# tusen-ai/SST

Hardware: AMD Instinct MI355X
Metric: LiDAR frames/sec (SST backbone fwd+bwd) at Waymo 0.32m voxels (higher is better)
Workload: dtype f32 (storage, accumulation, attention, LayerNorm, reductions: fp32; the dense products of the encoder layers from the EXACT three-way bf16 split of both fp32 operands, six bf16 MFMA products with fp32 accumulation - error vs float64 <= 2 x the fp32 matrix pipe's: tests/test_gpu_dense_f32x6.py)

## Files before the change

### sst_amd/csrc/wgrad_x6.hip

```cpp
#include <math.h>
#include <stdlib.h>
#include "common.h"

namespace {

typedef float f32x4 __attribute__((ext_vector_type(4)));
typedef float f32x2 __attribute__((ext_vector_type(2)));
typedef unsigned u32x4 __attribute__((ext_vector_type(4)));
typedef unsigned u32x2 __attribute__((ext_vector_type(2)));
typedef __bf16 bf16x8 __attribute__((ext_vector_type(8)));
typedef __bf16 bf16x2 __attribute__((ext_vector_type(2)));

__device__ __forceinline__ unsigned pack2(float lo, float hi) {
  const f32x2 v = {lo, hi};
  return __builtin_bit_cast(unsigned, __builtin_convertvector(v, bf16x2));
}
__device__ __forceinline__ float lo_f(unsigned p) { return __uint_as_float(p << 16); }
__device__ __forceinline__ float hi_f(unsigned p) { return __uint_as_float(p & 0xffff0000u); }
__device__ __forceinline__ f32x4 mma32(u32x4 a, u32x4 b, f32x4 c) {
  return __builtin_amdgcn_mfma_f32_16x16x32_bf16(__builtin_bit_cast(bf16x8, a), __builtin_bit_cast(bf16x8, b), c, 0, 0, 0);
}
__device__ __forceinline__ void split2(float a, float b, unsigned& p0, unsigned& p1, unsigned& p2) {
  p0 = pack2(a, b);
  const float ra = a - lo_f(p0), rb = b - hi_f(p0);
  p1 = pack2(ra, rb);
  p2 = pack2(ra - lo_f(p1), rb - hi_f(p1));
}

constexpr int kMaxProblems = 8;
constexpr int kTile = 128;
constexpr int kStep = 32;
constexpr int kTileLds = 1040;
constexpr int kImage = 8 * kTileLds;
constexpr int kStage = 2 * 3 * kImage;
constexpr int kLdsBytes = 2 * kStage;

struct x6_problem {
  const float* dy;
  const float* x;
  int64_t m, ld_dy, ld_x;
  int out, in;
  int tile0;
  int db_off;
  float* dw;
  float* db;
  const float* x_add_rows;
  const int32_t* x_add_index;
};
struct x6_group {
  x6_problem p[kMaxProblems];
  int n, tiles, slices;
  int64_t tokens_per_slice;
};

__global__ __launch_bounds__(512, 2) void wgrad_x6_k(const x6_group G, float* __restrict__ part, float* __restrict__ dbp) {
  extern __shared__ __attribute__((aligned(16))) unsigned char lds[];
  const int tid = threadIdx.x, lane = tid & 63, wave = tid >> 6;
  const int l15 = lane & 15, g = lane >> 4;
  const int tile = blockIdx.x / G.slices, slice = blockIdx.x - tile * G.slices;
  int pi = 0;
#pragma unroll
  for (int q = 1; q < kMaxProblems; ++q)
    if (q < G.n && tile >= G.p[q].tile0) pi = q;
  const x6_problem P = G.p[pi];
  const int tiles_k = P.in / kTile;
  const int tl = tile - P.tile0, tn = tl / tiles_k, tk = tl - tn * tiles_k;
  const int n0 = tn * kTile, k0 = tk * kTile;
  const int64_t t_begin = (int64_t)slice * G.tokens_per_slice;
  int64_t t_end = t_begin + G.tokens_per_slice;
  t_end = t_end < P.m ? t_end : P.m;

  const int op = tid >> 8, tq = (tid >> 5) & 7, cg = tid & 31;
  const float* src = op == 0 ? P.dy + n0 + 4 * cg : P.x + k0 + 4 * cg;
  const int64_t ld = op == 0 ? P.ld_dy : P.ld_x;
  const int st_off = (cg >> 2) * kTileLds + (tq & 1) * 512 + (tq >> 1) * 128 + (cg & 3) * 32;
  constexpr int kPf = 2;
  f32x4 rows[kPf][4];
  const int64_t t_last = t_end > 0 ? t_end - 1 : 0;
  const bool xadd = op == 1 && P.x_add_rows != nullptr;
  const float* addsrc = xadd ? P.x_add_rows + k0 + 4 * cg : nullptr;
  f32x4 prow[kPf][4];
  int32_t pidx[4] = {0, 0, 0, 0};
  auto load_idx = [&](int64_t t0) {
#pragma unroll
    for (int r = 0; r < 4; ++r) {
      int64_t t = t0 + 4 * tq + r;
      t = t < t_last ? t : t_last;
      pidx[r] = P.x_add_index[t];
    }
  };
  auto load_rows = [&](int64_t t0, f32x4 (&dst)[4], f32x4 (&pdst)[4]) {
#pragma unroll
    for (int r = 0; r < 4; ++r) {
      int64_t t = t0 + 4 * tq + r;
      t = t < t_last ? t : t_last;
      dst[r] = *(const f32x4*)(src + t * ld);
    }
    if (xadd) {
#pragma unroll
      for (int r = 0; r < 4; ++r) pdst[r] = *(const f32x4*)(addsrc + (int64_t)pidx[r] * P.in);
      load_idx(t0 + kStep);
    }
  };
  float bsum[4] = {0.f, 0.f, 0.f, 0.f};
  u32x4 img[3][2];
  auto split_col = [&](int e, int64_t t0, const f32x4 (&rws)[4], const f32x4 (&prw)[4]) {
    float v[4];
#pragma unroll
    for (int r = 0; r < 4; ++r) v[r] = (t0 + 4 * tq + r < t_end) ? (xadd ? rws[r][e] + prw[r][e] : rws[r][e]) : 0.f;
    if (op == 0) bsum[e] += (v[0] + v[1]) + (v[2] + v[3]);
    unsigned a0, a1, a2, b0, b1, b2;
    split2(v[0], v[1], a0, a1, a2);
    split2(v[2], v[3], b0, b1, b2);
    img[0][e >> 1][2 * (e & 1)] = a0;
    img[0][e >> 1][2 * (e & 1) + 1] = b0;
    img[1][e >> 1][2 * (e & 1)] = a1;
    img[1][e >> 1][2 * (e & 1) + 1] = b1;
    img[2][e >> 1][2 * (e & 1)] = a2;
    img[2][e >> 1][2 * (e & 1) + 1] = b2;
  };
  auto store_img = [&](int buf) {
    unsigned char* base = lds + buf * kStage + op * 3 * kImage + st_off;
#pragma unroll
    for (int im = 0; im < 3; ++im) {
      *(u32x4*)(base + im * kImage) = img[im][0];
      *(u32x4*)(base + im * kImage + 16) = img[im][1];
    }
  };
  const int wn = wave & 3, wk = wave >> 2;
  const int frag_off = g * 128 + l15 * 8;
  f32x4 acc[4][2], acl[4][2];
#pragma unroll
  for (int a = 0; a < 4; ++a)
#pragma unroll
    for (int b = 0; b < 2; ++b) acc[a][b] = acl[a][b] = (f32x4){0.f, 0.f, 0.f, 0.f};
  auto frag = [&](const unsigned char* image, int tile16) -> u32x4 {
    const unsigned char* p = image + tile16 * kTileLds + frag_off;
    const u32x2 lo = *(const u32x2*)p, hi = *(const u32x2*)(p + 512);
    return (u32x4){lo[0], lo[1], hi[0], hi[1]};
  };

  if (xadd) load_idx(t_begin);
#pragma unroll
  for (int u = 0; u < kPf; ++u) load_rows(t_begin + (int64_t)u * kStep, rows[u], prow[u]);
#pragma unroll
  for (int e = 0; e < 4; ++e) split_col(e, t_begin, rows[0], prow[0]);
  store_img(0);
  load_rows(t_begin + (int64_t)kPf * kStep, rows[0], prow[0]);
  __syncthreads();
  const int64_t n_steps = (t_end - t_begin + kStep - 1) / kStep;
  for (int64_t s0 = 0; s0 < n_steps; s0 += kPf) {
#pragma unroll
    for (int u = 0; u < kPf; ++u) {
      const int64_t s = s0 + u;
      if (s >= n_steps) break;
      const int64_t t1 = t_begin + (s + 1) * kStep;
      const unsigned char* dyi = lds + (u & 1) * kStage;
      const unsigned char* xi = dyi + 3 * kImage;
      u32x4 b0[2], b1[2], b2[2];
#pragma unroll
      for (int b = 0; b < 2; ++b) {
        b0[b] = frag(dyi, 2 * wn + b);
        b1[b] = frag(dyi + kImage, 2 * wn + b);
        b2[b] = frag(dyi + 2 * kImage, 2 * wn + b);
      }
#pragma unroll
      for (int a = 0; a < 4; ++a) {
        const u32x4 a0 = frag(xi, 4 * wk + a), a1 = frag(xi + kImage, 4 * wk + a), a2 = frag(xi + 2 * kImage, 4 * wk + a);
#pragma unroll
        for (int b = 0; b < 2; ++b) acl[a][b] = mma32(a2, b0[b], acl[a][b]);
#pragma unroll
        for (int b = 0; b < 2; ++b) acl[a][b] = mma32(a0, b2[b], acl[a][b]);
#pragma unroll
        for (int b = 0; b < 2; ++b) acl[a][b] = mma32(a1, b1[b], acl[a][b]);
#pragma unroll
        for (int b = 0; b < 2; ++b) acl[a][b] = mma32(a1, b0[b], acl[a][b]);
#pragma unroll
        for (int b = 0; b < 2; ++b) acl[a][b] = mma32(a0, b1[b], acl[a][b]);
#pragma unroll
        for (int b = 0; b < 2; ++b) acc[a][b] = mma32(a0, b0[b], acc[a][b]);
        split_col(a, t1, rows[(u + 1) % kPf], prow[(u + 1) % kPf]);
      }
      store_img((u + 1) & 1);
      load_rows(t1 + (int64_t)kPf * kStep, rows[(u + 1) % kPf], prow[(u + 1) % kPf]);
      __syncthreads();
    }
  }
#pragma unroll
  for (int a = 0; a < 4; ++a)
#pragma unroll
    for (int b = 0; b < 2; ++b) acc[a][b] += acl[a][b];
  float* dst = part + ((int64_t)tile * G.slices + slice) * (kTile * kTile);
#pragma unroll
  for (int a = 0; a < 4; ++a)
#pragma unroll
    for (int b = 0; b < 2; ++b)
      *(f32x4*)(dst + (32 * wn + 16 * b + l15) * kTile + 64 * wk + 16 * a + 4 * g) = acc[a][b];
  if (P.db_off >= 0 && tk == 0) {
    float* red = (float*)lds;
    if (op == 0) *(f32x4*)(red + tq * 128 + 4 * cg) = (f32x4){bsum[0], bsum[1], bsum[2], bsum[3]};
    __syncthreads();
    if (tid < 128) {
      float s = 0.f;
#pragma unroll
      for (int q = 0; q < 8; ++q) s += red[q * 128 + tid];
      dbp[((int64_t)P.db_off + n0 + tid) * G.slices + slice] = s;
    }
  }
}

struct x6_riders {
  sst_colsum_rider r[2];
  int n, blocks0;
};

constexpr int kRedQuads = 32, kRedGroups = 8;

__global__ __launch_bounds__(256) void wgrad_x6_reduce_k(const x6_group G, const float* __restrict__ part,
                                                         const float* __restrict__ dbp, int rider_blocks,
                                                         const x6_riders R) {
  __shared__ double red[kRedGroups][kRedQuads][4];
  if ((int)blockIdx.x < rider_blocks) {
    const int second = (int)blockIdx.x >= R.blocks0 ? 1 : 0;
    const sst_colsum_rider& J = R.r[second];
    const int rblk = (int)blockIdx.x - (second ? R.blocks0 : 0);
    float* fr = (float*)&red[0][0][0];
    const int cx = threadIdx.x & 31, gq = threadIdx.x >> 5;
    const int i = rblk * 32 + cx;
    float acc[4] = {0.f, 0.f, 0.f, 0.f};
    if (i < J.width) {
      const float* src = J.partials + i;
      for (int base = 0; base < J.nb; base += 512) {
        float v[16][4];
#pragma unroll
        for (int it = 0; it < 16; ++it)
#pragma unroll
          for (int j = 0; j < 4; ++j) {
            const int b = base + 32 * it + gq + 8 * j;
            v[it][j] = src[(int64_t)(b < J.nb ? b : J.nb - 1) * J.width];
          }
#pragma unroll
        for (int it = 0; it < 16; ++it)
#pragma unroll
          for (int j = 0; j < 4; ++j)
            if (base + 32 * it + gq + 8 * j < J.nb) acc[j] += v[it][j];
      }
    }
#pragma unroll
    for (int j = 0; j < 4; ++j) fr[(gq + 8 * j) * 33 + cx] = acc[j];
    __syncthreads();
    if (gq == 0 && i < J.width) {
      float t = 0.f;
#pragma unroll
      for (int k = 0; k < 32; ++k) t += fr[k * 33 + cx];
      if (i < J.split)
        J.out0[i] = t;
      else
        J.out1[i - J.split] = t;
    }
    return;
  }
  const int blk = (int)blockIdx.x - rider_blocks;
  const int ql = threadIdx.x & (kRedQuads - 1), sg = threadIdx.x / kRedQuads;
  const int64_t quad = (int64_t)blk * kRedQuads + ql;
  const int64_t tile = quad / (kTile * kTile / 4);
  const int e4 = (int)(quad - tile * (kTile * kTile / 4));
  double d0 = 0.0, d1 = 0.0, d2 = 0.0, d3 = 0.0;
  if (tile < G.tiles) {
    const float* src = part + tile * G.slices * (int64_t)(kTile * kTile) + 4 * e4;
#pragma unroll 8
    for (int q = sg; q < G.slices; q += kRedGroups) {
      const f32x4 v = *(const f32x4*)(src + (int64_t)q * (kTile * kTile));
      d0 += v[0], d1 += v[1], d2 += v[2], d3 += v[3];
    }
  }
  red[sg][ql][0] = d0, red[sg][ql][1] = d1, red[sg][ql][2] = d2, red[sg][ql][3] = d3;
  __syncthreads();
  if (sg == 0 && tile < G.tiles) {
    f32x4 s;
#pragma unroll
    for (int r = 0; r < 4; ++r) {
      double t = 0.0;
#pragma unroll
      for (int k = 0; k < kRedGroups; ++k) t += red[k][ql][r];
      s[r] = (float)t;
    }
    int pi = 0;
#pragma unroll
    for (int q = 1; q < kMaxProblems; ++q)
      if (q < G.n && tile >= G.p[q].tile0) pi = q;
    const int tiles_k = G.p[pi].in / kTile;
    const int tl = (int)tile - G.p[pi].tile0, tn = tl / tiles_k, tk = tl - tn * tiles_k;
    const int n = tn * kTile + e4 / 32, k = tk * kTile + (e4 % 32) * 4;
    *(f32x4*)(G.p[pi].dw + (int64_t)n * G.p[pi].in + k) = s;
  }
  const int64_t col = (int64_t)blk * 256 + threadIdx.x;
  int base = 0;
  for (int q = 0; q < G.n; ++q) {
    if (G.p[q].db_off < 0) continue;
    if (col >= base && col < base + G.p[q].out) {
      const float* src = dbp + ((int64_t)G.p[q].db_off + (col - base)) * G.slices;
      double s = 0.0;
      for (int i = 0; i < G.slices; ++i) s += src[i];
      G.p[q].db[col - base] = (float)s;
    }
    base += G.p[q].out;
  }
}

bool aligned16(const void* p) { return ((uintptr_t)p & 15) == 0; }

struct x6_plan {
  x6_group g;
  int64_t part_bytes, db_bytes;
};

bool make_plan(const sst_wgrad_problem_f32* pr, int n, x6_plan* plan) {
  if (!pr || n < 1 || n > kMaxProblems) return false;
  x6_group& G = plan->g;
  G.n = n;
  int tiles = 0, db_cols = 0;
  int64_t m = pr[0].m;
  for (int i = 0; i < n; ++i) {
    const sst_wgrad_problem_f32& p = pr[i];
    if (p.m != m || p.m < 1 || p.out < kTile || p.in < kTile || (p.out % kTile) || (p.in % kTile) || (p.ld_dy & 3) ||
        (p.ld_x & 3) || !p.dy || !p.x || !p.dw || !aligned16(p.dy) || !aligned16(p.x) || !aligned16(p.dw))
      return false;
    G.p[i].dy = p.dy;
    G.p[i].x = p.x;
    G.p[i].m = p.m;
    G.p[i].ld_dy = p.ld_dy;
    G.p[i].ld_x = p.ld_x;
    G.p[i].out = p.out;
    G.p[i].in = p.in;
    G.p[i].tile0 = tiles;
    G.p[i].db_off = p.db ? db_cols : -1;
    G.p[i].dw = p.dw;
    G.p[i].db = p.db;
    if ((p.x_add_rows != nullptr) != (p.x_add_index != nullptr) || (p.x_add_rows && !aligned16(p.x_add_rows))) return false;
    G.p[i].x_add_rows = p.x_add_rows;
    G.p[i].x_add_index = p.x_add_index;
    tiles += (p.out / kTile) * (p.in / kTile);
    if (p.db) db_cols += p.out;
  }
  G.tiles = tiles;
  int slices = (256 / tiles) & ~7;
  if (slices < 8) slices = 8;
  const int64_t max_slices = sst_div_up(m, (int64_t)kStep);
  while (slices > 8 && slices > max_slices) slices -= 8;
  G.slices = slices;
  G.tokens_per_slice = sst_align_up(sst_div_up(m, (int64_t)slices), (int64_t)kStep);
  plan->part_bytes = sst_align_up((int64_t)tiles * slices * kTile * kTile * 4, 256);
  plan->db_bytes = sst_align_up((int64_t)(db_cols > 0 ? db_cols : 1) * slices * 4, 256);
  return true;
}

}

extern "C" {

int64_t sst_weight_grad_group_f32x6_workspace_bytes(const sst_wgrad_problem_f32* problems, int n) {
  x6_plan plan;
  if (!make_plan(problems, n, &plan)) return SST_ERR_UNSUPPORTED;
  return plan.part_bytes + plan.db_bytes;
}

}

int sst_internal_weight_grad_group_f32x6(const sst_wgrad_problem_f32* problems, int n, void* d_workspace,
                                         const sst_colsum_rider* riders, int n_riders, void* stream) {
  x6_plan plan;
  if (!make_plan(problems, n, &plan)) return SST_ERR_UNSUPPORTED;
  if (!d_workspace || !aligned16(d_workspace)) return SST_ERR_ARG;
  hipStream_t st = (hipStream_t)stream;
  float* part = (float*)d_workspace;
  float* dbp = (float*)((char*)d_workspace + plan.part_bytes);
  static unsigned long long configured = 0;
  if (sst_first_use_on_device(&configured)) {
    SST_HIP(hipFuncSetAttribute((const void*)wgrad_x6_k, hipFuncAttributeMaxDynamicSharedMemorySize, kLdsBytes));
    sst_mark_device(&configured);
  }
  const int64_t quads = (int64_t)plan.g.tiles * (kTile * kTile / 4);
  const int tile_blocks = (int)sst_div_up(quads, (int64_t)kRedQuads);
  if (n_riders < 0 || n_riders > 2 || (n_riders > 0 && !riders)) return SST_ERR_ARG;
  x6_riders R;
  R.n = n_riders, R.blocks0 = 0;
  int extra = 0;
  for (int i = 0; i < n_riders; ++i) {
    const sst_colsum_rider& q = riders[i];
    if (!q.partials || q.nb < 1 || q.width < 1 || !q.out0 || !q.out1) return SST_ERR_ARG;
    R.r[i] = q;
    if (i == 0) R.blocks0 = (q.width + 31) / 32;
    extra += (q.width + 31) / 32;
  }
  hipLaunchKernelGGL(wgrad_x6_k, dim3((unsigned)(plan.g.tiles * plan.g.slices)), dim3(512), kLdsBytes, st, plan.g, part, dbp);
  hipLaunchKernelGGL(wgrad_x6_reduce_k, dim3((unsigned)(tile_blocks + extra)), dim3(256), 0, st, plan.g, part, dbp, extra, R);
  SST_LAUNCH_CHECK();
  return SST_OK;
}

extern "C" {

int sst_weight_grad_group_f32x6(const sst_wgrad_problem_f32* problems, int n, void* d_workspace, void* stream) {
  return sst_internal_weight_grad_group_f32x6(problems, n, d_workspace, nullptr, 0, stream);
}

}
```

Measured before the change: 97.71.

## Add warp-specialized wgrad x6 path and buffer loads, swizzled LDS, unmasked steps

Adds an optional producer/consumer variant of the x6 weight-gradient kernel in which 8 waves only run MFMAs while 4 extra waves load, split and stage both operands. It is selected by an environment variable and off by default. The default path also changes: full steps use buffer loads with scalar offsets and skip bounds masking, the LDS image layout is XOR-swizzled with permlane32 swaps so fragments load as one 16-byte read, and the bias sum runs only where it is needed. These aim to cut address arithmetic, masking and LDS bank conflicts, at the cost of code complexity and a separate ragged tail loop.

```diff
diff --git a/sst_amd/csrc/wgrad_x6.hip b/sst_amd/csrc/wgrad_x6.hip
--- a/sst_amd/csrc/wgrad_x6.hip
+++ b/sst_amd/csrc/wgrad_x6.hip
@@ -1,5 +1,6 @@
 #include <math.h>
 #include <stdlib.h>
+#include <type_traits>
 #include "common.h"
 
 namespace {
@@ -25,6 +26,15 @@
   const float ra = a - lo_f(p0), rb = b - hi_f(p0);
   p1 = pack2(ra, rb);
   p2 = pack2(ra - lo_f(p1), rb - hi_f(p1));
+}
+
+__device__ __forceinline__ __amdgpu_buffer_rsrc_t row_block(const void* p) {
+  const uint64_t v = (uint64_t)p;
+  const unsigned lo = __builtin_amdgcn_readfirstlane((unsigned)v), hi = __builtin_amdgcn_readfirstlane((unsigned)(v >> 32));
+  return __builtin_amdgcn_make_buffer_rsrc((void*)(((uint64_t)hi << 32) | lo), 0, 0x7fffffff, 0x00020000);
+}
+__device__ __forceinline__ f32x4 load16(__amdgpu_buffer_rsrc_t rs, unsigned voff, unsigned soff) {
+  return __builtin_bit_cast(f32x4, __builtin_amdgcn_raw_buffer_load_b128(rs, (int)voff, (int)soff, 0));
 }
 
 constexpr int kMaxProblems = 8;
@@ -34,6 +44,7 @@
 constexpr int kImage = 8 * kTileLds;
 constexpr int kStage = 2 * 3 * kImage;
 constexpr int kLdsBytes = 2 * kStage;
+constexpr bool kRolesDefault = false;
 
 struct x6_problem {
   const float* dy;
@@ -53,62 +64,101 @@
   int64_t tokens_per_slice;
 };
 
-__global__ __launch_bounds__(512, 2) void wgrad_x6_k(const x6_group G, float* __restrict__ part, float* __restrict__ dbp) {
+template <bool kRoles>
+__global__ __launch_bounds__(kRoles ? 768 : 512, kRoles ? 3 : 2) void wgrad_x6_k(const x6_group G, float* __restrict__ part,
+                                                                                 float* __restrict__ dbp) {
   extern __shared__ __attribute__((aligned(16))) unsigned char lds[];
-  const int tid = threadIdx.x, lane = tid & 63, wave = tid >> 6;
+  const int tid = threadIdx.x, lane = tid & 63;
+  const int wave = __builtin_amdgcn_readfirstlane(tid >> 6);
   const int l15 = lane & 15, g = lane >> 4;
-  const int tile = blockIdx.x / G.slices, slice = blockIdx.x - tile * G.slices;
+  const int tile = __builtin_amdgcn_readfirstlane(blockIdx.x / G.slices), slice = blockIdx.x - tile * G.slices;
   int pi = 0;
 #pragma unroll
   for (int q = 1; q < kMaxProblems; ++q)
     if (q < G.n && tile >= G.p[q].tile0) pi = q;
   const x6_problem P = G.p[pi];
   const int tiles_k = P.in / kTile;
-  const int tl = tile - P.tile0, tn = tl / tiles_k, tk = tl - tn * tiles_k;
+  const int tl = tile - P.tile0, tn = __builtin_amdgcn_readfirstlane(tl / tiles_k), tk = tl - tn * tiles_k;
   const int n0 = tn * kTile, k0 = tk * kTile;
   const int64_t t_begin = (int64_t)slice * G.tokens_per_slice;
   int64_t t_end = t_begin + G.tokens_per_slice;
   t_end = t_end < P.m ? t_end : P.m;
 
-  const int op = tid >> 8, tq = (tid >> 5) & 7, cg = tid & 31;
-  const float* src = op == 0 ? P.dy + n0 + 4 * cg : P.x + k0 + 4 * cg;
-  const int64_t ld = op == 0 ? P.ld_dy : P.ld_x;
-  const int st_off = (cg >> 2) * kTileLds + (tq & 1) * 512 + (tq >> 1) * 128 + (cg & 3) * 32;
+  constexpr int kOps = kRoles ? 2 : 1;
+  const int op0 = kRoles ? 0 : wave >> 2;
+  const int tq = (tid >> 5) & 7, cg = tid & 31;
+  const float* opbase[kOps];
+  int64_t ld[kOps];
+  unsigned voff[kOps][4];
+  __amdgpu_buffer_rsrc_t rs[kOps];
+#pragma unroll
+  for (int o = 0; o < kOps; ++o) {
+    opbase[o] = op0 + o == 0 ? P.dy + n0 : P.x + k0;
+    ld[o] = op0 + o == 0 ? P.ld_dy : P.ld_x;
+    rs[o] = row_block(opbase[o] + t_begin * ld[o]);
+#pragma unroll
+    for (int r = 0; r < 4; ++r) voff[o][r] = (unsigned)((4 * tq + r) * ld[o] * 4 + 16 * cg);
+  }
+  const int st_col = 4 * (cg & 3) + 2 * (tq & 1);
+  const int st_off = (cg >> 2) * kTileLds + (tq >> 1) * 256 + (st_col ^ ((st_col & 8) >> 2)) * 16;
   constexpr int kPf = 2;
-  f32x4 rows[kPf][4];
+  constexpr int kPp = kRoles ? 1 : kPf;
+  f32x4 rows[kPf][kOps][4];
   const int64_t t_last = t_end > 0 ? t_end - 1 : 0;
-  const bool xadd = op == 1 && P.x_add_rows != nullptr;
+  constexpr int oX = kRoles ? 1 : 0;
+  const bool xadd = op0 + oX == 1 && P.x_add_rows != nullptr;
   const float* addsrc = xadd ? P.x_add_rows + k0 + 4 * cg : nullptr;
-  f32x4 prow[kPf][4];
+  f32x4 prow[kPp][4];
   int32_t pidx[4] = {0, 0, 0, 0};
-  auto load_idx = [&](int64_t t0) {
+  const __amdgpu_buffer_rsrc_t idx_rs = row_block(xadd ? P.x_add_index + t_begin : nullptr);
+  auto load_idx = [&](auto full, int64_t j) {
+    const int64_t t0 = t_begin + j * kStep;
 #pragma unroll
     for (int r = 0; r < 4; ++r) {
-      int64_t t = t0 + 4 * tq + r;
-      t = t < t_last ? t : t_last;
-      pidx[r] = P.x_add_index[t];
-    }
-  };
-  auto load_rows = [&](int64_t t0, f32x4 (&dst)[4], f32x4 (&pdst)[4]) {
-#pragma unroll
-    for (int r = 0; r < 4; ++r) {
-      int64_t t = t0 + 4 * tq + r;
-      t = t < t_last ? t : t_last;
-      dst[r] = *(const f32x4*)(src + t * ld);
-    }
+      if constexpr (decltype(full)::value) {
+        pidx[r] = (int32_t)__builtin_amdgcn_raw_buffer_load_b32(idx_rs, 4 * (4 * tq + r), (int)(j * kStep * 4), 0);
+      } else {
+        int64_t t = t0 + 4 * tq + r;
+        t = t < t_last ? t : t_last;
+        pidx[r] = P.x_add_index[t];
+      }
+    }
+  };
+  auto load_rows = [&](auto full, int64_t j, f32x4 (&dst)[kOps][4]) {
+    const int64_t t0 = t_begin + j * kStep;
+#pragma unroll
+    for (int o = 0; o < kOps; ++o) {
+      if constexpr (decltype(full)::value) {
+#pragma unroll
+        for (int r = 0; r < 4; ++r) dst[o][r] = load16(rs[o], voff[o][r], (unsigned)(j * kStep * ld[o] * 4));
+      } else {
+#pragma unroll
+        for (int r = 0; r < 4; ++r) {
+          int64_t t = t0 + 4 * tq + r;
+          t = t < t_last ? t : t_last;
+          dst[o][r] = *(const f32x4*)(opbase[o] + t * ld[o] + 4 * cg);
+        }
+      }
+    }
+  };
+  auto load_pos = [&](auto full, int64_t j, f32x4 (&pdst)[4]) {
     if (xadd) {
 #pragma unroll
       for (int r = 0; r < 4; ++r) pdst[r] = *(const f32x4*)(addsrc + (int64_t)pidx[r] * P.in);
-      load_idx(t0 + kStep);
-    }
-  };
+      load_idx(full, j + 1);
+    }
+  };
+  const bool want_b = P.db_off >= 0 && tk == 0;
   float bsum[4] = {0.f, 0.f, 0.f, 0.f};
   u32x4 img[3][2];
-  auto split_col = [&](int e, int64_t t0, const f32x4 (&rws)[4], const f32x4 (&prw)[4]) {
+  auto split_col = [&](auto full, int e, int o, int64_t j, const f32x4 (&rws)[4], const f32x4 (&prw)[4]) {
     float v[4];
 #pragma unroll
-    for (int r = 0; r < 4; ++r) v[r] = (t0 + 4 * tq + r < t_end) ? (xadd ? rws[r][e] + prw[r][e] : rws[r][e]) : 0.f;
-    if (op == 0) bsum[e] += (v[0] + v[1]) + (v[2] + v[3]);
+    for (int r = 0; r < 4; ++r) {
+      v[r] = (o == oX && xadd) ? rws[r][e] + prw[r][e] : rws[r][e];
+      if constexpr (!decltype(full)::value) v[r] = (t_begin + j * kStep + 4 * tq + r < t_end) ? v[r] : 0.f;
+    }
+    if (op0 + o == 0 && want_b) bsum[e] += (v[0] + v[1]) + (v[2] + v[3]);
     unsigned a0, a1, a2, b0, b1, b2;
     split2(v[0], v[1], a0, a1, a2);
     split2(v[2], v[3], b0, b1, b2);
@@ -119,86 +169,146 @@
     img[2][e >> 1][2 * (e & 1)] = a2;
     img[2][e >> 1][2 * (e & 1) + 1] = b2;
   };
-  auto store_img = [&](int buf) {
-    unsigned char* base = lds + buf * kStage + op * 3 * kImage + st_off;
+  auto store_img = [&](int buf, int o) {
+    unsigned char* base = lds + buf * kStage + (op0 + o) * 3 * kImage + st_off;
 #pragma unroll
     for (int im = 0; im < 3; ++im) {
-      *(u32x4*)(base + im * kImage) = img[im][0];
-      *(u32x4*)(base + im * kImage + 16) = img[im][1];
-    }
-  };
-  const int wn = wave & 3, wk = wave >> 2;
-  const int frag_off = g * 128 + l15 * 8;
+      u32x2 w[4];
+#pragma unroll
+      for (int i = 0; i < 4; ++i) w[i] = __builtin_amdgcn_permlane32_swap(img[im][0][i], img[im][1][i], false, false);
+      *(u32x4*)(base + im * kImage) = (u32x4){w[0][0], w[1][0], w[0][1], w[1][1]};
+      *(u32x4*)(base + im * kImage + 16) = (u32x4){w[2][0], w[3][0], w[2][1], w[3][1]};
+    }
+  };
+  const int wn = wave & 3, wk = (wave >> 2) & 1;
+  const int frag_off = g * 256 + (l15 ^ ((l15 & 8) >> 2)) * 16;
   f32x4 acc[4][2], acl[4][2];
-#pragma unroll
-  for (int a = 0; a < 4; ++a)
-#pragma unroll
-    for (int b = 0; b < 2; ++b) acc[a][b] = acl[a][b] = (f32x4){0.f, 0.f, 0.f, 0.f};
+  auto zero_acc = [&]() {
+#pragma unroll
+    for (int a = 0; a < 4; ++a)
+#pragma unroll
+      for (int b = 0; b < 2; ++b) acc[a][b] = acl[a][b] = (f32x4){0.f, 0.f, 0.f, 0.f};
+  };
   auto frag = [&](const unsigned char* image, int tile16) -> u32x4 {
     const unsigned char* p = image + tile16 * kTileLds + frag_off;
-    const u32x2 lo = *(const u32x2*)p, hi = *(const u32x2*)(p + 512);
-    return (u32x4){lo[0], lo[1], hi[0], hi[1]};
-  };
-
-  if (xadd) load_idx(t_begin);
-#pragma unroll
-  for (int u = 0; u < kPf; ++u) load_rows(t_begin + (int64_t)u * kStep, rows[u], prow[u]);
-#pragma unroll
-  for (int e = 0; e < 4; ++e) split_col(e, t_begin, rows[0], prow[0]);
-  store_img(0);
-  load_rows(t_begin + (int64_t)kPf * kStep, rows[0], prow[0]);
-  __syncthreads();
+    return *(const u32x4*)p;
+  };
+  auto multiply = [&](int buf, auto&& between) {
+    const unsigned char* dyi = lds + buf * kStage;
+    const unsigned char* xi = dyi + 3 * kImage;
+    u32x4 b0[2], b1[2], b2[2];
+#pragma unroll
+    for (int b = 0; b < 2; ++b) {
+      b0[b] = frag(dyi, 2 * wn + b);
+      b1[b] = frag(dyi + kImage, 2 * wn + b);
+      b2[b] = frag(dyi + 2 * kImage, 2 * wn + b);
+    }
+#pragma unroll
+    for (int a = 0; a < 4; ++a) {
+      const u32x4 a0 = frag(xi, 4 * wk + a), a1 = frag(xi + kImage, 4 * wk + a), a2 = frag(xi + 2 * kImage, 4 * wk + a);
+#pragma unroll
+      for (int b = 0; b < 2; ++b) acl[a][b] = mma32(a2, b0[b], acl[a][b]);
+#pragma unroll
+      for (int b = 0; b < 2; ++b) acl[a][b] = mma32(a0, b2[b], acl[a][b]);
+#pragma unroll
+      for (int b = 0; b < 2; ++b) acl[a][b] = mma32(a1, b1[b], acl[a][b]);
+#pragma unroll
+      for (int b = 0; b < 2; ++b) acl[a][b] = mma32(a1, b0[b], acl[a][b]);
+#pragma unroll
+      for (int b = 0; b < 2; ++b) acl[a][b] = mma32(a0, b1[b], acl[a][b]);
+#pragma unroll
+      for (int b = 0; b < 2; ++b) acc[a][b] = mma32(a0, b0[b], acc[a][b]);
+      between(a);
+    }
+  };
+  auto stage_cols = [&](auto full, int u, int64_t s, int o, int e) {
+    split_col(full, e, o, s + 1, rows[(u + 1) % kPf][o], prow[(u + 1) % kPp]);
+  };
+  auto stage_refill = [&](auto full, int u, int64_t s) {
+    load_rows(full, s + 1 + kPf, rows[(u + 1) % kPf]);
+    load_pos(full, s + 1 + kPp, prow[(u + 1) % kPp]);
+  };
+  const std::false_type ragged;
+  const std::true_type whole;
+  auto stage_first = [&]() {
+    if (xadd) load_idx(ragged, 0);
+#pragma unroll
+    for (int u = 0; u < kPf; ++u) load_rows(ragged, u, rows[u]);
+#pragma unroll
+    for (int u = 0; u < kPp; ++u) load_pos(ragged, u, prow[u]);
+#pragma unroll
+    for (int o = 0; o < kOps; ++o) {
+#pragma unroll
+      for (int e = 0; e < 4; ++e) split_col(ragged, e, o, 0, rows[0][o], prow[0]);
+      store_img(0, o);
+    }
+    load_rows(ragged, kPf, rows[0]);
+    load_pos(ragged, kPp, prow[0]);
+  };
   const int64_t n_steps = (t_end - t_begin + kStep - 1) / kStep;
-  for (int64_t s0 = 0; s0 < n_steps; s0 += kPf) {
-#pragma unroll
-    for (int u = 0; u < kPf; ++u) {
-      const int64_t s = s0 + u;
-      if (s >= n_steps) break;
-      const int64_t t1 = t_begin + (s + 1) * kStep;
-      const unsigned char* dyi = lds + (u & 1) * kStage;
-      const unsigned char* xi = dyi + 3 * kImage;
-      u32x4 b0[2], b1[2], b2[2];
-#pragma unroll
-      for (int b = 0; b < 2; ++b) {
-        b0[b] = frag(dyi, 2 * wn + b);
-        b1[b] = frag(dyi + kImage, 2 * wn + b);
-        b2[b] = frag(dyi + 2 * kImage, 2 * wn + b);
+  const int64_t max_ld = P.ld_dy > P.ld_x ? P.ld_dy : P.ld_x;
+  const bool offsets_fit = P.ld_dy >= 0 && P.ld_x >= 0 && (G.tokens_per_slice + kStep) * max_ld * 4 < (int64_t(1) << 31);
+  const int64_t n_full = t_end > t_begin && offsets_fit ? (t_end - t_begin) / kStep : 0;
+  const int64_t n_fast = n_full > 2 + kPf ? (n_full - 2 - kPf) / kPf * kPf : 0;
+  auto steps = [&](auto&& body) {
+    __syncthreads();
+    for (int64_t s0 = 0; s0 < n_fast; s0 += kPf) {
+#pragma unroll
+      for (int u = 0; u < kPf; ++u) {
+        body(whole, u, s0 + u);
+        __syncthreads();
       }
-#pragma unroll
-      for (int a = 0; a < 4; ++a) {
-        const u32x4 a0 = frag(xi, 4 * wk + a), a1 = frag(xi + kImage, 4 * wk + a), a2 = frag(xi + 2 * kImage, 4 * wk + a);
-#pragma unroll
-        for (int b = 0; b < 2; ++b) acl[a][b] = mma32(a2, b0[b], acl[a][b]);
-#pragma unroll
-        for (int b = 0; b < 2; ++b) acl[a][b] = mma32(a0, b2[b], acl[a][b]);
-#pragma unroll
-        for (int b = 0; b < 2; ++b) acl[a][b] = mma32(a1, b1[b], acl[a][b]);
-#pragma unroll
-        for (int b = 0; b < 2; ++b) acl[a][b] = mma32(a1, b0[b], acl[a][b]);
-#pragma unroll
-        for (int b = 0; b < 2; ++b) acl[a][b] = mma32(a0, b1[b], acl[a][b]);
-#pragma unroll
-        for (int b = 0; b < 2; ++b) acc[a][b] = mma32(a0, b0[b], acc[a][b]);
-        split_col(a, t1, rows[(u + 1) % kPf], prow[(u + 1) % kPf]);
+    }
+    for (int64_t s0 = n_fast; s0 < n_steps; s0 += kPf) {
+#pragma unroll
+      for (int u = 0; u < kPf; ++u) {
+        if (s0 + u >= n_steps) break;
+        body(ragged, u, s0 + u);
+        __syncthreads();
       }
-      store_img((u + 1) & 1);
-      load_rows(t1 + (int64_t)kPf * kStep, rows[(u + 1) % kPf], prow[(u + 1) % kPf]);
-      __syncthreads();
-    }
-  }
-#pragma unroll
-  for (int a = 0; a < 4; ++a)
-#pragma unroll
-    for (int b = 0; b < 2; ++b) acc[a][b] += acl[a][b];
-  float* dst = part + ((int64_t)tile * G.slices + slice) * (kTile * kTile);
-#pragma unroll
-  for (int a = 0; a < 4; ++a)
-#pragma unroll
-    for (int b = 0; b < 2; ++b)
-      *(f32x4*)(dst + (32 * wn + 16 * b + l15) * kTile + 64 * wk + 16 * a + 4 * g) = acc[a][b];
-  if (P.db_off >= 0 && tk == 0) {
+    }
+  };
+  auto write_tile = [&]() {
+#pragma unroll
+    for (int a = 0; a < 4; ++a)
+#pragma unroll
+      for (int b = 0; b < 2; ++b) acc[a][b] += acl[a][b];
+    float* dst = part + ((int64_t)tile * G.slices + slice) * (kTile * kTile);
+#pragma unroll
+    for (int a = 0; a < 4; ++a)
+#pragma unroll
+      for (int b = 0; b < 2; ++b)
+        *(f32x4*)(dst + (32 * wn + 16 * b + l15) * kTile + 64 * wk + 16 * a + 4 * g) = acc[a][b];
+  };
+  if constexpr (!kRoles) {
+    zero_acc();
+    stage_first();
+    steps([&](auto full, int u, int64_t s) {
+      multiply(u & 1, [&](int a) { stage_cols(full, u, s, 0, a); });
+      store_img((u + 1) & 1, 0);
+      stage_refill(full, u, s);
+    });
+    write_tile();
+  } else if (wave < 8) {
+    zero_acc();
+    steps([&](auto, int u, int64_t) { multiply(u & 1, [](int) {}); });
+    write_tile();
+  } else {
+    stage_first();
+    steps([&](auto full, int u, int64_t s) {
+#pragma unroll
+      for (int o = 0; o < kOps; ++o) {
+#pragma unroll
+        for (int e = 0; e < 4; ++e) stage_cols(full, u, s, o, e);
+        store_img((u + 1) & 1, o);
+        __builtin_amdgcn_sched_barrier(0);
+      }
+      stage_refill(full, u, s);
+    });
+  }
+  if (want_b) {
     float* red = (float*)lds;
-    if (op == 0) *(f32x4*)(red + tq * 128 + 4 * cg) = (f32x4){bsum[0], bsum[1], bsum[2], bsum[3]};
+    if (kRoles ? wave >= 8 : op0 == 0) *(f32x4*)(red + tq * 128 + 4 * cg) = (f32x4){bsum[0], bsum[1], bsum[2], bsum[3]};
     __syncthreads();
     if (tid < 128) {
       float s = 0.f;
@@ -375,9 +485,14 @@
   hipStream_t st = (hipStream_t)stream;
   float* part = (float*)d_workspace;
   float* dbp = (float*)((char*)d_workspace + plan.part_bytes);
+  static const bool roles = [] {
+    const char* e = getenv("SST_WGRAD_X6_ROLES");
+    return e ? atoi(e) != 0 : kRolesDefault;
+  }();
   static unsigned long long configured = 0;
   if (sst_first_use_on_device(&configured)) {
-    SST_HIP(hipFuncSetAttribute((const void*)wgrad_x6_k, hipFuncAttributeMaxDynamicSharedMemorySize, kLdsBytes));
+    SST_HIP(hipFuncSetAttribute((const void*)wgrad_x6_k<false>, hipFuncAttributeMaxDynamicSharedMemorySize, kLdsBytes));
+    SST_HIP(hipFuncSetAttribute((const void*)wgrad_x6_k<true>, hipFuncAttributeMaxDynamicSharedMemorySize, kLdsBytes));
     sst_mark_device(&configured);
   }
   const int64_t quads = (int64_t)plan.g.tiles * (kTile * kTile / 4);
@@ -393,7 +508,11 @@
     if (i == 0) R.blocks0 = (q.width + 31) / 32;
     extra += (q.width + 31) / 32;
   }
-  hipLaunchKernelGGL(wgrad_x6_k, dim3((unsigned)(plan.g.tiles * plan.g.slices)), dim3(512), kLdsBytes, st, plan.g, part, dbp);
+  const dim3 grid((unsigned)(plan.g.tiles * plan.g.slices));
+  if (roles)
+    hipLaunchKernelGGL(wgrad_x6_k<true>, grid, dim3(768), kLdsBytes, st, plan.g, part, dbp);
+  else
+    hipLaunchKernelGGL(wgrad_x6_k<false>, grid, dim3(512), kLdsBytes, st, plan.g, part, dbp);
   hipLaunchKernelGGL(wgrad_x6_reduce_k, dim3((unsigned)(tile_blocks + extra)), dim3(256), 0, st, plan.g, part, dbp, extra, R);
   SST_LAUNCH_CHECK();
   return SST_OK;
```

New measurement: 99.18 (median of 4 runs). +1.5%, better.

## Specialize wgrad x6 kernel per wave role and add bounds-free interior loop

Applied to the files above, without the earlier changes.

Splits the weight-gradient x6 kernel into a templated per-role body (dy with bias, dy plain, x plain, x with positional add), chosen per wave with a uniform branch. The roles are compile-time constants, so per-thread selects, unused prefetch registers and bias sums drop out of each specialization. It also adds an interior main loop that uses 32-bit byte offsets and advancing pointers with no token clamping or tail masking, falling back to the generic path only for the edge steps. The risk is more code size, possible divergence in how the compiler schedules the two loops, and a new restriction that positional-add problems must have in == kTile.

```diff
diff --git a/sst_amd/csrc/wgrad_x6.hip b/sst_amd/csrc/wgrad_x6.hip
--- a/sst_amd/csrc/wgrad_x6.hip
+++ b/sst_amd/csrc/wgrad_x6.hip
@@ -1,5 +1,6 @@
 #include <math.h>
 #include <stdlib.h>
+#include <type_traits>
 #include "common.h"
 
 namespace {
@@ -53,34 +54,33 @@
   int64_t tokens_per_slice;
 };
 
-__global__ __launch_bounds__(512, 2) void wgrad_x6_k(const x6_group G, float* __restrict__ part, float* __restrict__ dbp) {
-  extern __shared__ __attribute__((aligned(16))) unsigned char lds[];
-  const int tid = threadIdx.x, lane = tid & 63, wave = tid >> 6;
+enum { kDyBias, kDyPlain, kXPlain, kXPos };
+
+template <int kRole>
+__device__ __forceinline__ void wgrad_x6_tile(const x6_group& G, const x6_problem& P, const int tile, const int slice, const int tn,
+                                              const int tk, const int wave, float* __restrict__ part, float* __restrict__ dbp,
+                                              unsigned char* lds) {
+  constexpr int op = kRole == kDyBias || kRole == kDyPlain ? 0 : 1;
+  constexpr bool kPos = kRole == kXPos, kBias = kRole == kDyBias;
+  const int tid = threadIdx.x, lane = tid & 63;
   const int l15 = lane & 15, g = lane >> 4;
-  const int tile = blockIdx.x / G.slices, slice = blockIdx.x - tile * G.slices;
-  int pi = 0;
-#pragma unroll
-  for (int q = 1; q < kMaxProblems; ++q)
-    if (q < G.n && tile >= G.p[q].tile0) pi = q;
-  const x6_problem P = G.p[pi];
-  const int tiles_k = P.in / kTile;
-  const int tl = tile - P.tile0, tn = tl / tiles_k, tk = tl - tn * tiles_k;
   const int n0 = tn * kTile, k0 = tk * kTile;
   const int64_t t_begin = (int64_t)slice * G.tokens_per_slice;
   int64_t t_end = t_begin + G.tokens_per_slice;
   t_end = t_end < P.m ? t_end : P.m;
 
-  const int op = tid >> 8, tq = (tid >> 5) & 7, cg = tid & 31;
-  const float* src = op == 0 ? P.dy + n0 + 4 * cg : P.x + k0 + 4 * cg;
+  const int tq = (tid >> 5) & 7, cg = tid & 31;
+  const float* src = op == 0 ? P.dy + n0 : P.x + k0;
   const int64_t ld = op == 0 ? P.ld_dy : P.ld_x;
   const int st_off = (cg >> 2) * kTileLds + (tq & 1) * 512 + (tq >> 1) * 128 + (cg & 3) * 32;
   constexpr int kPf = 2;
   f32x4 rows[kPf][4];
   const int64_t t_last = t_end > 0 ? t_end - 1 : 0;
-  const bool xadd = op == 1 && P.x_add_rows != nullptr;
+  constexpr bool xadd = kPos;
   const float* addsrc = xadd ? P.x_add_rows + k0 + 4 * cg : nullptr;
-  f32x4 prow[kPf][4];
+  f32x4 prow[kPos ? kPf : 1][4];
   int32_t pidx[4] = {0, 0, 0, 0};
+
   auto load_idx = [&](int64_t t0) {
 #pragma unroll
     for (int r = 0; r < 4; ++r) {
@@ -94,7 +94,7 @@
     for (int r = 0; r < 4; ++r) {
       int64_t t = t0 + 4 * tq + r;
       t = t < t_last ? t : t_last;
-      dst[r] = *(const f32x4*)(src + t * ld);
+      dst[r] = *(const f32x4*)(src + 4 * cg + t * ld);
     }
     if (xadd) {
 #pragma unroll
@@ -102,13 +102,30 @@
       load_idx(t0 + kStep);
     }
   };
+  const uint32_t ldb = (uint32_t)ld * 4u;
+  const uint32_t voff = (uint32_t)(4 * tq) * ldb + 16u * (uint32_t)cg;
+  const uint32_t ioff = 16u * (uint32_t)tq;
+  auto load_rows_interior = [&](const unsigned char* fp, const unsigned char* ip, f32x4 (&dst)[4], f32x4 (&pdst)[4]) {
+#pragma unroll
+    for (int r = 0; r < 4; ++r) dst[r] = *(const f32x4*)(fp + (size_t)r * ldb + voff);
+    if (xadd) {
+#pragma unroll
+      for (int r = 0; r < 4; ++r) pdst[r] = *(const f32x4*)(addsrc + (int64_t)pidx[r] * P.in);
+#pragma unroll
+      for (int r = 0; r < 4; ++r) pidx[r] = *(const int32_t*)(ip + 4 * r + ioff);
+    }
+  };
   float bsum[4] = {0.f, 0.f, 0.f, 0.f};
   u32x4 img[3][2];
-  auto split_col = [&](int e, int64_t t0, const f32x4 (&rws)[4], const f32x4 (&prw)[4]) {
+  auto split_col = [&](auto interior, int e, int64_t t0, const f32x4 (&rws)[4], const f32x4 (&prw)[4]) {
     float v[4];
 #pragma unroll
-    for (int r = 0; r < 4; ++r) v[r] = (t0 + 4 * tq + r < t_end) ? (xadd ? rws[r][e] + prw[r][e] : rws[r][e]) : 0.f;
-    if (op == 0) bsum[e] += (v[0] + v[1]) + (v[2] + v[3]);
+    for (int r = 0; r < 4; ++r) {
+      v[r] = rws[r][e];
+      if constexpr (kPos) v[r] += prw[r][e];
+      if constexpr (!decltype(interior)::value) v[r] = (t0 + 4 * tq + r < t_end) ? v[r] : 0.f;
+    }
+    if constexpr (kBias) bsum[e] += (v[0] + v[1]) + (v[2] + v[3]);
     unsigned a0, a1, a2, b0, b1, b2;
     split2(v[0], v[1], a0, a1, a2);
     split2(v[2], v[3], b0, b1, b2);
@@ -139,51 +156,77 @@
     const u32x2 lo = *(const u32x2*)p, hi = *(const u32x2*)(p + 512);
     return (u32x4){lo[0], lo[1], hi[0], hi[1]};
   };
+  auto step = [&](auto interior, int u, int64_t t1, const unsigned char* fp, const unsigned char* ip) {
+    const unsigned char* dyi = lds + (u & 1) * kStage;
+    const unsigned char* xi = dyi + 3 * kImage;
+    u32x4 b0[2], b1[2], b2[2];
+#pragma unroll
+    for (int b = 0; b < 2; ++b) {
+      b0[b] = frag(dyi, 2 * wn + b);
+      b1[b] = frag(dyi + kImage, 2 * wn + b);
+      b2[b] = frag(dyi + 2 * kImage, 2 * wn + b);
+    }
+#pragma unroll
+    for (int a = 0; a < 4; ++a) {
+      const u32x4 a0 = frag(xi, 4 * wk + a), a1 = frag(xi + kImage, 4 * wk + a), a2 = frag(xi + 2 * kImage, 4 * wk + a);
+#pragma unroll
+      for (int b = 0; b < 2; ++b) acl[a][b] = mma32(a2, b0[b], acl[a][b]);
+#pragma unroll
+      for (int b = 0; b < 2; ++b) acl[a][b] = mma32(a0, b2[b], acl[a][b]);
+#pragma unroll
+      for (int b = 0; b < 2; ++b) acl[a][b] = mma32(a1, b1[b], acl[a][b]);
+#pragma unroll
+      for (int b = 0; b < 2; ++b) acl[a][b] = mma32(a1, b0[b], acl[a][b]);
+#pragma unroll
+      for (int b = 0; b < 2; ++b) acl[a][b] = mma32(a0, b1[b], acl[a][b]);
+#pragma unroll
+      for (int b = 0; b < 2; ++b) acc[a][b] = mma32(a0, b0[b], acc[a][b]);
+      split_col(interior, a, t1, rows[(u + 1) % kPf], prow[kPos ? (u + 1) % kPf : 0]);
+    }
+    store_img((u + 1) & 1);
+    if constexpr (decltype(interior)::value)
+      load_rows_interior(fp, ip, rows[(u + 1) % kPf], prow[kPos ? (u + 1) % kPf : 0]);
+    else
+      load_rows(t1 + (int64_t)kPf * kStep, rows[(u + 1) % kPf], prow[kPos ? (u + 1) % kPf : 0]);
+    __syncthreads();
+  };
+  constexpr std::true_type kInterior{};
+  constexpr std::false_type kGeneric{};
 
   if (xadd) load_idx(t_begin);
 #pragma unroll
-  for (int u = 0; u < kPf; ++u) load_rows(t_begin + (int64_t)u * kStep, rows[u], prow[u]);
-#pragma unroll
-  for (int e = 0; e < 4; ++e) split_col(e, t_begin, rows[0], prow[0]);
+  for (int u = 0; u < kPf; ++u) load_rows(t_begin + (int64_t)u * kStep, rows[u], prow[kPos ? u : 0]);
+#pragma unroll
+  for (int e = 0; e < 4; ++e) split_col(kGeneric, e, t_begin, rows[0], prow[0]);
   store_img(0);
   load_rows(t_begin + (int64_t)kPf * kStep, rows[0], prow[0]);
   __syncthreads();
-  const int64_t n_steps = (t_end - t_begin + kStep - 1) / kStep;
-  for (int64_t s0 = 0; s0 < n_steps; s0 += kPf) {
+  const int64_t n_tok = t_end > t_begin ? t_end - t_begin : 0;
+  const int64_t n_steps = (n_tok + kStep - 1) / kStep, n_full = n_tok / kStep;
+  int64_t n_int = n_full - (kPf + 1);
+  n_int = (n_int < 0 || ld >= (1 << 24) || ld < 0) ? 0 : n_int & ~(int64_t)1;
+  {
+    const unsigned char* fp = (const unsigned char*)(src + (t_begin + (int64_t)(kPf + 1) * kStep) * ld);
+    const unsigned char* ip = (const unsigned char*)(P.x_add_index + t_begin);
+    const size_t fstep = (size_t)kStep * ldb;
+    for (int64_t s0 = 0; s0 < n_int; s0 += kPf) {
+#pragma unroll
+      for (int u = 0; u < kPf; ++u) {
+        const int64_t s = s0 + u;
+        int64_t si = s + 2 + kPf;
+        si = si < n_full ? si : n_full - 1;
+        step(kInterior, u, t_begin + (s + 1) * kStep, fp, ip + si * (4 * kStep));
+        fp += fstep;
+      }
+    }
+  }
+  if (xadd && n_int > 0) load_idx(t_begin + (n_int + 1 + kPf) * kStep);
+  for (int64_t s0 = n_int; s0 < n_steps; s0 += kPf) {
 #pragma unroll
     for (int u = 0; u < kPf; ++u) {
       const int64_t s = s0 + u;
       if (s >= n_steps) break;
-      const int64_t t1 = t_begin + (s + 1) * kStep;
-      const unsigned char* dyi = lds + (u & 1) * kStage;
-      const unsigned char* xi = dyi + 3 * kImage;
-      u32x4 b0[2], b1[2], b2[2];
-#pragma unroll
-      for (int b = 0; b < 2; ++b) {
-        b0[b] = frag(dyi, 2 * wn + b);
-        b1[b] = frag(dyi + kImage, 2 * wn + b);
-        b2[b] = frag(dyi + 2 * kImage, 2 * wn + b);
-      }
-#pragma unroll
-      for (int a = 0; a < 4; ++a) {
-        const u32x4 a0 = frag(xi, 4 * wk + a), a1 = frag(xi + kImage, 4 * wk + a), a2 = frag(xi + 2 * kImage, 4 * wk + a);
-#pragma unroll
-        for (int b = 0; b < 2; ++b) acl[a][b] = mma32(a2, b0[b], acl[a][b]);
-#pragma unroll
-        for (int b = 0; b < 2; ++b) acl[a][b] = mma32(a0, b2[b], acl[a][b]);
-#pragma unroll
-        for (int b = 0; b < 2; ++b) acl[a][b] = mma32(a1, b1[b], acl[a][b]);
-#pragma unroll
-        for (int b = 0; b < 2; ++b) acl[a][b] = mma32(a1, b0[b], acl[a][b]);
-#pragma unroll
-        for (int b = 0; b < 2; ++b) acl[a][b] = mma32(a0, b1[b], acl[a][b]);
-#pragma unroll
-        for (int b = 0; b < 2; ++b) acc[a][b] = mma32(a0, b0[b], acc[a][b]);
-        split_col(a, t1, rows[(u + 1) % kPf], prow[(u + 1) % kPf]);
-      }
-      store_img((u + 1) & 1);
-      load_rows(t1 + (int64_t)kPf * kStep, rows[(u + 1) % kPf], prow[(u + 1) % kPf]);
-      __syncthreads();
+      step(kGeneric, u, t_begin + (s + 1) * kStep, nullptr, nullptr);
     }
   }
 #pragma unroll
@@ -198,7 +241,7 @@
       *(f32x4*)(dst + (32 * wn + 16 * b + l15) * kTile + 64 * wk + 16 * a + 4 * g) = acc[a][b];
   if (P.db_off >= 0 && tk == 0) {
     float* red = (float*)lds;
-    if (op == 0) *(f32x4*)(red + tq * 128 + 4 * cg) = (f32x4){bsum[0], bsum[1], bsum[2], bsum[3]};
+    if constexpr (kBias) *(f32x4*)(red + tq * 128 + 4 * cg) = (f32x4){bsum[0], bsum[1], bsum[2], bsum[3]};
     __syncthreads();
     if (tid < 128) {
       float s = 0.f;
@@ -206,6 +249,29 @@
       for (int q = 0; q < 8; ++q) s += red[q * 128 + tid];
       dbp[((int64_t)P.db_off + n0 + tid) * G.slices + slice] = s;
     }
+  }
+}
+
+__global__ __launch_bounds__(512, 2) void wgrad_x6_k(const x6_group G, float* __restrict__ part, float* __restrict__ dbp) {
+  extern __shared__ __attribute__((aligned(16))) unsigned char lds[];
+  const int tile = blockIdx.x / G.slices, slice = blockIdx.x - tile * G.slices;
+  int pi = 0;
+#pragma unroll
+  for (int q = 1; q < kMaxProblems; ++q)
+    if (q < G.n && tile >= G.p[q].tile0) pi = q;
+  const x6_problem P = G.p[pi];
+  const int tiles_k = P.in / kTile;
+  const int tl = tile - P.tile0, tn = tl / tiles_k, tk = tl - tn * tiles_k;
+  const int wave = __builtin_amdgcn_readfirstlane(threadIdx.x >> 6);
+  if (wave < 4) {
+    if (P.db_off >= 0 && tk == 0)
+      wgrad_x6_tile<kDyBias>(G, P, tile, slice, tn, tk, wave, part, dbp, lds);
+    else
+      wgrad_x6_tile<kDyPlain>(G, P, tile, slice, tn, tk, wave, part, dbp, lds);
+  } else if (P.x_add_rows != nullptr) {
+    wgrad_x6_tile<kXPos>(G, P, tile, slice, tn, tk, wave, part, dbp, lds);
+  } else {
+    wgrad_x6_tile<kXPlain>(G, P, tile, slice, tn, tk, wave, part, dbp, lds);
   }
 }
 
@@ -338,6 +404,7 @@
     G.p[i].dw = p.dw;
     G.p[i].db = p.db;
     if ((p.x_add_rows != nullptr) != (p.x_add_index != nullptr) || (p.x_add_rows && !aligned16(p.x_add_rows))) return false;
+    if (p.x_add_rows && p.in != kTile) return false;
     G.p[i].x_add_rows = p.x_add_rows;
     G.p[i].x_add_index = p.x_add_index;
     tiles += (p.out / kTile) * (p.in / kTile);
```

Result: no change. 92.64 before, 94.72 after, median of 6 (+2.2%).
